# gillett-hernandez/rust-pathtracer

Measured on AMD Instinct MI355X. Metric: Msamples/s (paths×spp/s) Cornell box 1024², max_bounces=8; 1/2/4/8 GPU, higher is better.
Workload: dtype f32

## Files before the change

### include/pt_api.h

```cpp
#ifndef PT_API_H
#define PT_API_H

#include <stddef.h>
#include <stdint.h>

#ifdef __cplusplus
extern "C" {
#endif

typedef int32_t pt_status;
enum {
    PT_OK = 0,
    PT_ERR_INVALID_ARGUMENT = 1,
    PT_ERR_NO_DEVICE = 2,
    PT_ERR_OUT_OF_MEMORY = 3,
    PT_ERR_UNSUPPORTED = 4,
    PT_ERR_DEVICE = 5
};

enum { PT_TAG_MATERIAL = 0, PT_TAG_LIGHT = 1, PT_TAG_CAMERA = 2 };
#define PT_MATERIAL_ID(tag, index) ((((uint32_t)(tag)) << 16) | ((uint32_t)(index) & 0xffffu))
#define PT_MATERIAL_TAG(id) (((id) >> 16) & 0x3u)
#define PT_MATERIAL_INDEX(id) ((id) & 0xffffu)
#define PT_MATERIAL_NONE 0xffffffffu
// ... 152 lines not shown
    PT_TUNE_NO_CORE_LDS = 1u << 1,
    PT_TUNE_NO_PARK = 1u << 2,
    PT_TUNE_NO_LIVE_LIST = 1u << 3,
    PT_TUNE_EXACT_SLAB = 1u << 4,
    PT_TUNE_NO_CULL = 1u << 5,
    PT_TUNE_NO_SWEEP = 1u << 6,
    PT_TUNE_NO_MESH_SWEEP = 1u << 7,
    PT_TUNE_NO_KNOWN_LIGHT = 1u << 8,
    PT_TUNE_GENERAL_FORMS = 1u << 9,
    PT_TUNE_NO_FUSE = 1u << 10,
    PT_TUNE_NO_STAGE_TIMING = 1u << 11,
    PT_TUNE_MULTI_RCCL = 1u << 12,
    PT_TUNE_NO_ONE_LIGHT = 1u << 14,
    PT_TUNE_NO_CONVEX = 1u << 15,
    PT_TUNE_NO_MESH_SHORTCUTS = 1u << 16,
    PT_TUNE_NO_AXIS_SCAN = 1u << 13
};
typedef struct pt_tuning {
    uint32_t flags;
    uint32_t batch_slots;
    uint32_t blocks_per_cu;
    uint32_t park_blocks_per_cu;
    int32_t park_dynamic;
    uint32_t shade_form;
    uint32_t lds_all_limit;
    uint32_t multi_virtual;
    uint32_t walk_evict_below;
    uint32_t walk_search_below;
    uint32_t park_block;
    uint32_t light_prepass_max;
    uint32_t top_evict_below;
// ... 81 lines not shown
```

### rust-pathtracer_amd/api.py

```python
import ctypes as C
import numpy as np

PT_OK = 0
PT_ERR_UNSUPPORTED = 4
TAG_MATERIAL, TAG_LIGHT, TAG_CAMERA = 0, 1, 2
MATERIAL_NONE = 0xFFFFFFFF

CURVE_LINEAR, CURVE_TABULATED, CURVE_CAUCHY, CURVE_EXPONENTIAL, CURVE_INV_EXPONENTIAL, CURVE_BLACKBODY, CURVE_CONST = range(7)
INTERP_LINEAR, INTERP_NEAREST, INTERP_CUBIC = range(3)
TEXTURE1, TEXTURE4 = 1, 4
MATERIAL_LAMBERTIAN, MATERIAL_GGX, MATERIAL_DIFFUSE_LIGHT, MATERIAL_SHARP_LIGHT, MATERIAL_PASSTHROUGH = range(5)
MEDIUM_HG, MEDIUM_RAYLEIGH = range(2)
SIDED_FORWARD, SIDED_REVERSE, SIDED_DUAL = range(3)
SHAPE_RECT, SHAPE_SPHERE, SHAPE_DISK, SHAPE_MESH = range(4)
AXIS_X, AXIS_Y, AXIS_Z = range(3)
ENV_CONSTANT, ENV_SUN, ENV_HDR = range(3)


def material_id(tag, index):
    return ((tag & 3) << 16) | (index & 0xFFFF)


class Curve(C.Structure):
    _fields_ = [("kind", C.c_int32), ("mode", C.c_int32), ("p0", C.c_float), ("p1", C.c_float),
# ... 114 lines not shown
    _fields_ = [("max_chain", C.c_uint32), ("alpha_max", C.c_float), ("reserved", C.c_uint32 * 2)]


class Profile(C.Structure):
    _fields_ = [("bounce_rays", C.c_uint64), ("shadow_rays", C.c_uint64), ("light_rays", C.c_uint64),
                ("camera_rays", C.c_uint64), ("env_hits", C.c_uint64), ("seconds", C.c_double),
                ("kernel_seconds", C.c_double * 8), ("kernel_launches", C.c_uint64 * 8), ("stage_items", C.c_uint64 * 8)]

    def as_dict(self):
        return {"bounce_rays": self.bounce_rays, "shadow_rays": self.shadow_rays, "light_rays": self.light_rays,
                "camera_rays": self.camera_rays, "env_hits": self.env_hits, "seconds": self.seconds,
                "kernel_seconds": list(self.kernel_seconds), "kernel_launches": list(self.kernel_launches), "stage_items": list(self.stage_items)}


TUNE_NO_LDS, TUNE_NO_CORE_LDS, TUNE_NO_PARK, TUNE_NO_LIVE_LIST, TUNE_EXACT_SLAB, TUNE_NO_CULL, TUNE_NO_SWEEP, TUNE_NO_MESH_SWEEP, TUNE_NO_KNOWN_LIGHT, \
    TUNE_GENERAL_FORMS, TUNE_NO_FUSE, TUNE_NO_STAGE_TIMING, TUNE_MULTI_RCCL, TUNE_NO_AXIS_SCAN, TUNE_NO_ONE_LIGHT, TUNE_NO_CONVEX, TUNE_NO_MESH_SHORTCUTS = (1 << i for i in range(17))


class Tuning(C.Structure):
    _fields_ = [("flags", C.c_uint32), ("batch_slots", C.c_uint32), ("blocks_per_cu", C.c_uint32), ("park_blocks_per_cu", C.c_uint32),
                ("park_dynamic", C.c_int32), ("shade_form", C.c_uint32), ("lds_all_limit", C.c_uint32), ("multi_virtual", C.c_uint32),
                ("walk_evict_below", C.c_uint32), ("walk_search_below", C.c_uint32), ("park_block", C.c_uint32), ("light_prepass_max", C.c_uint32), ("top_evict_below", C.c_uint32), ("group_evict_below", C.c_uint32), ("reserved", C.c_uint32 * 2)]


class OutputDesc(C.Structure):
    _fields_ = [("width", C.c_uint32), ("height", C.c_uint32), ("tonemap", C.c_int32), ("luminance_only", C.c_int32),
                ("exposure", C.c_float), ("key_value", C.c_float), ("white_point", C.c_float), ("colorspace", C.c_int32),
                ("factor", C.c_float)]


TONEMAP_CLAMP, TONEMAP_REINHARD0, TONEMAP_REINHARD1 = range(3)
# ... 739 lines not shown
```

### rust-pathtracer_amd/csrc/pt_engine.hip

```cpp
#include <hip/hip_runtime.h>

#include <dlfcn.h>
#include <rccl/rccl.h>

#include <algorithm>
#include <chrono>
#include <condition_variable>
#include <functional>
#include <mutex>
#include <thread>
#include <cstdio>
#include <cstring>
#include <string>
#include <vector>

#include "pt_kernels.h"
#include "../../include/pt_adaptive.h"
#include "../../include/pt_spectral.h"
#include "../../include/pt_api.h"
#include "../../include/pt_debug.h"
#include "../../include/pt_denoise.h"
#include "pt_adaptive_select.h"
#include "pt_spectral_launch.h"
#include "pt_spectral_rules.h"
// ... 263 lines not shown
    }
    struct pt_resident_info info() const { struct pt_resident_info i; i.width = width; i.height = height; i.bins = bins; i.parts = parts; return i; }
};

struct pt_scene {
    pth::HostScene host;
    pt_tuning tuning;
    MultiSetup multi;
    uint32_t* d_blob = nullptr;
    float* d_tex = nullptr;
    uint32_t blob_words = 0;
    int lds_mode = 0;
    uint32_t lacks = 0;
    int device = 0, num_cus = 0;
    DeviceBuffers buf;
    AdaptiveBuffers adaptive;
    std::vector<hipEvent_t> events;
    GrowBuf film_cache;
    GrowBuf spectral_cache;
    bool spectral_valid = false;
    uint32_t spectral_width = 0, spectral_height = 0, spectral_bins = 0;
    std::vector<pt_scene*> spectral_shards;
    std::vector<uint32_t> shard_px;
    GrowBuf shard_packed;
    ResidentSet resident;
    GrowBuf assemble_staging, assemble_px;
    GrowBuf project_cache;
    std::vector<pt_scene*> replicas;
};

namespace {
bool scene_has_mesh(const std::vector<uint32_t>& blob) {
// ... 5 lines not shown
std::string g_device_info;

pt_status no_device() { return fail(PT_ERR_NO_DEVICE, "no HIP device available: the product path has no CPU fallback"); }
pt_status ensure_device() {
    int n = 0;
    hipError_t e = hipGetDeviceCount(&n);
    if (e != hipSuccess || n == 0) return no_device();
    return PT_OK;
}

uint32_t segment_capacity(uint32_t n, int grid) {
    uint32_t c = (n + (uint32_t)grid - 1) / (uint32_t)grid;
    return (c + 63u) & ~63u;
}

pt_status ensure_buffers(pt_scene* sc, uint32_t capacity, uint32_t light_samples, size_t n_pixels, int grid, uint32_t nl, uint32_t park_block) {
    DeviceBuffers& b = sc->buf;
    uint32_t total = segment_capacity(capacity, grid) * (uint32_t)grid;
    if (b.capacity < total || b.light_samples < light_samples || b.grid != grid || b.nl < nl || b.park_block < park_block) {
        hipFree(b.paths_a); hipFree(b.paths_b); hipFree(b.hits); hipFree(b.shadow); hipFree(b.energy); hipFree(b.counts); hipFree(b.block_stats); hipFree(b.park);
        b.paths_a = b.paths_b = b.hits = b.shadow = b.counts = b.park = nullptr; b.energy = nullptr; b.block_stats = nullptr; b.capacity = 0;
        uint32_t ls = light_samples > b.light_samples ? light_samples : b.light_samples;
        uint32_t nlmax = nl > b.nl ? nl : b.nl;
        size_t path_fields = nlmax == 4 ? Layout<4>::path_fields : Layout<1>::path_fields;
        size_t sh_fields = nlmax == 4 ? Layout<4>::shadow_queue_fields(ls ? ls : 1) : Layout<1>::shadow_queue_fields(ls ? ls : 1);
        HIP_TRY(hipMalloc(&b.paths_a, sizeof(uint32_t) * path_fields * total));
        HIP_TRY(hipMalloc(&b.paths_b, sizeof(uint32_t) * path_fields * total));
        HIP_TRY(hipMalloc(&b.hits, sizeof(uint32_t) * (size_t)HS_FIELDS * total));
        HIP_TRY(hipMalloc(&b.shadow, sizeof(uint32_t) * sh_fields * total));
        HIP_TRY(hipMalloc(&b.energy, sizeof(float) * (size_t)(nlmax + 1u) * total));
        b.nl = nlmax;
        HIP_TRY(hipMalloc(&b.counts, sizeof(uint32_t) * 4 * (size_t)grid));
        HIP_TRY(hipMalloc(&b.block_stats, sizeof(unsigned long long) * BS_FIELDS * (size_t)grid));
        const bool no_table = sc->host.blob[PT_HDR_SWEEP_OFF] == 0 || (sc->host.blob[PT_HDR_FLAGS] & PT_FLAG_NO_SWEEP);
        if ((sc->host.blob[PT_HDR_FLAGS] & PT_FLAG_SWEEP_WALKS) || no_table)
            HIP_TRY(hipMalloc(&b.park, sizeof(uint32_t) * kParkFields * (kParkCap / (kBlock / 64)) * (park_block / 64) * (size_t)grid));
        b.park_block = park_block;
        if (!b.unit_counters) HIP_TRY(hipMalloc(&b.unit_counters, sizeof(uint32_t) * kUnitCounters));
        b.capacity = total; b.light_samples = ls; b.grid = grid;
    }
    if (b.pixel_capacity < n_pixels) {
        hipFree(b.pixels); b.pixels = nullptr;
        HIP_TRY(hipMalloc(&b.pixels, sizeof(uint32_t) * n_pixels));
        b.pixel_capacity = n_pixels;
    }
    return PT_OK;
}

pt_status ensure_adaptive_buffers(pt_scene* sc, size_t n_pixels) {
    AdaptiveBuffers& a = sc->adaptive;
    if (a.pixels >= n_pixels) return PT_OK;
    a.release();
    const size_t blocks = (n_pixels + kBlock - 1) / kBlock;
    HIP_TRY(hipMalloc(&a.counts, sizeof(uint32_t) * n_pixels));
    HIP_TRY(hipMalloc(&a.lists[0], sizeof(uint32_t) * n_pixels));
// ... 194 lines not shown
                         : (env_prob != 0.0f || tn.shade_form == 2) ? PT_SHADE_FULL : (has_ggx || certs || tn.shade_form == 1) ? PT_SHADE_NO_ENV : PT_SHADE_LEAN;
    cfg.certs = certs;
    uint32_t live_list = ((trav_form == PT_FORM_SWEEP || trav_form == PT_FORM_WALK || trav_form == PT_FORM_ANY) && shade_form == PT_SHADE_LEAN && !(tn.flags & PT_TUNE_NO_LIVE_LIST)) ? 1u : 0u;
#ifdef PT_EXPERIMENTS
    if (cfg.live_lists || getenv("PT_AMD_EXP_SHADOW")) live_list = 0u;
#endif
    const uint32_t camera_record = (shade_form == PT_SHADE_LEAN || shade_form == PT_SHADE_FULL || shade_form == PT_SHADE_MEDIUM) ? 1u : 0u;
    cfg.fuse = !(tn.flags & PT_TUNE_NO_FUSE) && (!hero || PT_FUSE_HERO) && trav_form == PT_FORM_SWEEP && shade_form == PT_SHADE_LEAN && (cfg.lacks & PT_SCENE_NO_XF) != 0;
    const uint32_t path_fields = hero ? Layout<4>::path_fields : (rd.medium_aware ? (uint32_t)PS_FIELDS + 2u : Layout<1>::path_fields);
    const uint32_t item_fields = hero ? Layout<4>::shadow_queue_fields(rd.light_samples ? rd.light_samples : 1) : Layout<1>::shadow_queue_fields(rd.light_samples ? rd.light_samples : 1);
    *plan = RenderPlan{capacity, grid, hero, park_block, park_block_extend, trav_form, shade_form, park_dynamic, park_big, cfg, live_list, camera_record,
                       path_fields, item_fields};
    return PT_OK;
}

pt_status read_profile(pt_scene* sc, const RenderPlan& plan, uint64_t camera_rays, uint64_t accumulated_pixels, const double* stage_ms, const uint64_t* stage_launches,
                       uint32_t rounds, double seconds, pt_profile* profile) {
    memset(profile, 0, sizeof(*profile));
    std::vector<unsigned long long> bs((size_t)plan.grid * BS_FIELDS);
    HIP_TRY(hipMemcpy(bs.data(), sc->buf.block_stats, sizeof(unsigned long long) * bs.size(), hipMemcpyDeviceToHost));
    unsigned long long c[BS_FIELDS] = {0, 0, 0, 0, 0, 0};
    for (int g = 0; g < plan.grid; ++g) for (int k = 0; k < BS_FIELDS; ++k) c[k] += bs[(size_t)g * BS_FIELDS + k];
    profile->camera_rays = camera_rays;
    profile->bounce_rays = c[BS_VERTICES] + camera_rays;
    profile->shadow_rays = c[BS_SHADOW_RAYS];
    profile->env_hits = c[BS_ENV_HITS];
    profile->seconds = seconds;
    for (int i = 0; i < ST_COUNT; ++i) { profile->kernel_seconds[i] = stage_ms[i] * 1e-3; profile->kernel_launches[i] = stage_launches[i]; }
    profile->stage_items[ST_GENERATE] = camera_rays; profile->stage_items[ST_EXTEND] = c[BS_SEGMENTS]; profile->stage_items[ST_SHADE] = c[BS_SEGMENTS];
    profile->stage_items[ST_SHADOW] = c[BS_ITEMS]; profile->stage_items[ST_ACCUMULATE] = accumulated_pixels;
    profile->stage_items[6] = (uint64_t)plan.cfg.park_block;
    profile->stage_items[7] = plan.camera_record;
    profile->stage_items[5] = c[BS_MEDIUM_DROPS];
    profile->kernel_launches[5] = rounds;
    return PT_OK;
}

pt_status render_impl(pt_scene* sc, const pt_render_desc* rdp, float* d_film, hipStream_t stream, pt_profile* profile, const RenderJob& job) {
    if (!sc || !rdp || !d_film) return fail(PT_ERR_INVALID_ARGUMENT, "null argument");
    pt_render_desc rd;
    std::string err;
    if (!pth::normalize_render_desc(*rdp, (uint32_t)sc->host.cameras.size(), &rd, &err)) return fail(PT_ERR_INVALID_ARGUMENT, err);
    HIP_TRY(hipSetDevice(sc->device));

    const pt_adaptive_desc* adaptive = job.adaptive;
    std::vector<uint32_t> own_list;
    if (!job.shard_list) own_list = pth::shard_pixels(rd.width, rd.height, rd.tile_width, rd.tile_height, rd.shard_index, rd.shard_count);
    const std::vector<uint32_t>& pixels = job.shard_list ? *job.shard_list : own_list;
    RenderPlan plan;
    pt_status st = plan_render(sc, rd, job, pixels, stream, &plan);
    if (st != PT_OK) return st;
    const uint32_t capacity = plan.capacity;
    const int grid = plan.grid, trav_form = plan.trav_form, shade_form = plan.shade_form;
    const bool hero = plan.hero, park_dynamic = plan.park_dynamic;
    LaunchCfg cfg = plan.cfg;

    st = ensure_buffers(sc, capacity, rd.light_samples, pixels.size() ? pixels.size() : 1, grid, (hero || rd.medium_aware) ? 4u : 1u, plan.park_block);
    if (st != PT_OK) return st;
    DeviceBuffers& b = sc->buf;
    if ((trav_form == PT_FORM_PARKED || trav_form == PT_FORM_PARKED_WALK) && !b.park) return fail(PT_ERR_DEVICE, "internal: a parked traversal form without the parked kernels' scratch");
    if (adaptive) {
        const size_t film_pixels = (size_t)rd.width * rd.height;
        st = ensure_adaptive_buffers(sc, film_pixels);
        if (st != PT_OK) return st;
        if (!pixels.empty()) HIP_TRY(hipMemcpyAsync(sc->adaptive.lists[0], pixels.data(), sizeof(uint32_t) * pixels.size(), hipMemcpyHostToDevice, stream));
        if (job.shard_list && !pixels.empty()) HIP_TRY(hipMemcpyAsync(b.pixels, pixels.data(), sizeof(uint32_t) * pixels.size(), hipMemcpyHostToDevice, stream));
        HIP_TRY(hipMemsetAsync(sc->adaptive.stats, 0, sizeof(double) * 2 * film_pixels, stream));
        if (pixels.size() < film_pixels) HIP_TRY(hipMemsetAsync(sc->adaptive.counts, 0, sizeof(uint32_t) * film_pixels, stream));
    } else if (!pixels.empty()) HIP_TRY(hipMemcpyAsync(b.pixels, pixels.data(), sizeof(uint32_t) * pixels.size(), hipMemcpyHostToDevice, stream));
    HIP_TRY(hipMemsetAsync(d_film, 0, sizeof(float) * 4 * (size_t)rd.width * rd.height, stream));
    if (job.d_spectral) HIP_TRY(hipMemsetAsync(job.d_spectral, 0, sizeof(float) * (size_t)job.spectral_bins * rd.width * rd.height, stream));
    HIP_TRY(hipMemsetAsync(b.block_stats, 0, sizeof(unsigned long long) * BS_FIELDS * (size_t)grid, stream));

    RenderParams rp;
    memset(&rp, 0, sizeof(rp));
    rp.seed = rd.seed; rp.width = rd.width; rp.height = rd.height;
    rp.min_bounces = rd.min_bounces; rp.max_bounces = rd.max_bounces; rp.light_samples = rd.light_samples; rp.only_direct = rd.only_direct;
    rp.wavelength_lo = rd.wavelength_lo; rp.wavelength_span = rd.wavelength_hi - rd.wavelength_lo;
    rp.spp = adaptive ? adaptive->max_samples : rd.spp; rp.range_end = rd.first_sample + rd.sample_count;
    rp.normalize = (!adaptive && rd.first_sample == 0 && rd.sample_count == rd.spp) ? 1u : 0u;
    rp.phase = rd.phase_samples;
    rp.camera = pth::camera_params(sc->host.cameras[rd.camera_index], (float)rd.width / (float)rd.height);
    rp.energy_stride = b.capacity;
    rp.live_list = plan.live_list; rp.camera_record = plan.camera_record;

    const pt_tuning& tn = sc->tuning;
    const SceneArgs sargs{sc->d_blob, sc->blob_words, sc->d_tex, marginal_lds_bytes(sc->host.blob.data(), cfg.lds_bytes)};
    const uint32_t bounce_limit = rd.only_direct ? 1u : rd.max_bounces;
    const bool timing = !(tn.flags & PT_TUNE_NO_STAGE_TIMING);
    double stage_ms[ST_COUNT] = {0, 0, 0, 0, 0};
    uint64_t stage_launches[ST_COUNT] = {0, 0, 0, 0, 0};
    Queue qa{b.paths_a, b.capacity, plan.path_fields}, qb{b.paths_b, b.capacity, plan.path_fields}, qh{b.hits, b.capacity, HS_FIELDS}, qs{b.shadow, b.capacity, plan.item_fields};
    uint32_t* live[2] = {b.counts, b.counts + grid};
    uint32_t* nshadow = b.counts + 2 * grid;

    HIP_TRY(hipStreamSynchronize(stream));
    const auto t0 = std::chrono::steady_clock::now();
    std::vector<int> event_stage;
    auto event_at = [&](size_t k) -> bool {
        while (sc->events.size() <= k) { hipEvent_t e; if (hipEventCreate(&e) != hipSuccess) return false; sc->events.push_back(e); }
        return hipEventRecord(sc->events[k], stream) == hipSuccess;
    };
    bool events_ok = timing && event_at(0);
    auto timed = [&](int stage, auto&& fn) {
        fn();
        if (events_ok) { events_ok = event_at(event_stage.size() + 1); if (events_ok) event_stage.push_back(stage); }
        stage_launches[stage]++;
    };

    uint64_t camera_rays = 0, accumulated_pixels = 0;
    hipError_t spectral_error = hipSuccess;
    auto run_passes = [&](const uint32_t* d_list, uint32_t n_list, uint32_t first_sample, uint32_t sample_count, double* d_stats) -> pt_status {
        if (camera_rays != 0 && events_ok) { events_ok = event_at(event_stage.size() + 1); if (events_ok) event_stage.push_back(-1); }
        rp.range_end = first_sample + sample_count;
        std::vector<pth::Pass> passes = pth::plan_passes(n_list, first_sample, sample_count, capacity, rd.phase_samples);
        for (const pth::Pass& pass : passes) {
            accumulated_pixels += pass.pixel_count;
            rp.chunk_pixels = pass.pixel_count; rp.first_sample = pass.first_sample; rp.pass_samples = pass.sample_count;
            uint32_t n = pass.pixel_count * pass.sample_count;
            if (n > b.capacity) return fail(PT_ERR_DEVICE, "internal: a pass of " + std::to_string(n) + " slots exceeds the queue capacity " + std::to_string(b.capacity));
            uint32_t seg_cap = segment_capacity(n, grid);
            camera_rays += n;
            const uint32_t* d_px = d_list + pass.pixel_begin;
            if (park_dynamic) {
                HIP_TRY(hipMemsetAsync(b.unit_counters, 0, sizeof(uint32_t) * kUnitCounters, stream));
                if (events_ok) { events_ok = event_at(event_stage.size() + 1); if (events_ok) event_stage.push_back(-1); }
            }
            timed(ST_GENERATE, [&] {
                if (hero) hipLaunchKernelGGL(k_generate<4>, dim3(grid), dim3(kBlock), 0, stream, rp, d_px, qa, b.energy, n, seg_cap, live[0]);
                else hipLaunchKernelGGL(k_generate<1>, dim3(grid), dim3(kBlock), 0, stream, rp, d_px, qa, b.energy, n, seg_cap, live[0]);
            });
            for (uint32_t bounce = 0; bounce < bounce_limit; ++bounce) {
                Queue qin = (bounce & 1) ? qb : qa, qout = (bounce & 1) ? qa : qb;
                uint32_t *cin = live[bounce & 1], *cout = live[(bounce + 1) & 1];
                if (park_dynamic) cfg.unit_counter = b.unit_counters + 2 * bounce;
                cfg.path_marks = (bounce > 0 && !rd.medium_aware && (sc->host.blob[PT_HDR_FLAGS] & PT_FLAG_CONVEX)) ? sc->host.blob[PT_HDR_CONVEX_INST] : 0u;
                if (!cfg.fuse) timed(ST_EXTEND, [&] { launch_extend(cfg, trav_form, sargs, qin, qh, seg_cap, cin, b.park); });
                if (park_dynamic) cfg.unit_counter = b.unit_counters + 2 * bounce + 1;
                timed(ST_SHADE, [&] { launch_shade(cfg, hero ? 4 : 1, shade_form, sargs, rp, bounce, d_px, qin, qh, qout, qs, b.energy, seg_cap, cin, cout, nshadow, b.block_stats); });
                if (rd.light_samples > 0)
                    timed(ST_SHADOW, [&] { launch_shadow(cfg, trav_form, hero ? 4 : 1, shade_form == PT_SHADE_FULL || shade_form == PT_SHADE_MEDIUM, sargs, rd.light_samples, qs, b.energy, b.capacity, rp.live_list ? (seg_cap | kShadowListed) : seg_cap, nshadow, b.park, qh); });
            }
            timed(ST_ACCUMULATE, [&] {
                if (d_stats && hero) hipLaunchKernelGGL(k_accumulate_stats<4>, dim3(grid), dim3(kBlock), 0, stream, rp, d_px, b.energy, d_film, d_stats);
                else if (d_stats) hipLaunchKernelGGL(k_accumulate_stats<1>, dim3(grid), dim3(kBlock), 0, stream, rp, d_px, b.energy, d_film, d_stats);
                else if (hero) hipLaunchKernelGGL(k_accumulate<4>, dim3(grid), dim3(kBlock), 0, stream, rp, d_px, b.energy, d_film);
                else hipLaunchKernelGGL(k_accumulate<1>, dim3(grid), dim3(kBlock), 0, stream, rp, d_px, b.energy, d_film);
                if (job.d_spectral && spectral_error == hipSuccess)
                    spectral_error = ptk::launch_accumulate_spectral(hero ? 4 : 1, grid, stream, rp, d_px, b.energy, job.d_spectral, job.spectral_bins, rd.width * rd.height);
            });
            if (spectral_error != hipSuccess) return fail(PT_ERR_DEVICE, std::string("k_accumulate_spectral: ") + hipGetErrorString(spectral_error));
        }
        return PT_OK;
    };
    uint32_t rounds = 0;
    st = adaptive ? adaptive_rounds(sc, rd, *adaptive, stream, d_film, (uint32_t)pixels.size(), run_passes, &rounds, job.node, job.node_index)
                  : run_passes(b.pixels, (uint32_t)pixels.size(), rd.first_sample, rd.sample_count, nullptr);
    if (st != PT_OK) return st;
    if (adaptive && job.d_spectral)
        hipLaunchKernelGGL(k_adaptive_finish_spectral, dim3(sc->num_cus * 4), dim3(kBlock), 0, stream, rd.width * rd.height, job.spectral_bins, sc->adaptive.counts, job.d_spectral);
    HIP_TRY(hipGetLastError());
    HIP_TRY(hipStreamSynchronize(stream));
    auto t1 = std::chrono::steady_clock::now();
    for (size_t k = 0; k < event_stage.size(); ++k) {
        float ms = 0.0f;
        if (event_stage[k] >= 0 && hipEventElapsedTime(&ms, sc->events[k], sc->events[k + 1]) == hipSuccess) stage_ms[event_stage[k]] += ms;
    }
    if (profile) return read_profile(sc, plan, camera_rays, accumulated_pixels, stage_ms, stage_launches, rounds, std::chrono::duration<double>(t1 - t0).count(), profile);
    return PT_OK;
}

pt_status probe_material(pt_scene* sc, int mode, uint32_t record, size_t n, const float* lambda, const float* a, size_t a_w, const float* b, size_t b_w,
                         float* f, float* wo, float* pdf) {
    HIP_TRY(hipSetDevice(sc->device));
    DevBuf dl, da, db, df, dwo, dp;
    size_t m = n ? n : 1;
    HIP_TRY(dl.alloc(4 * m)); HIP_TRY(da.alloc(4 * m * 3)); HIP_TRY(db.alloc(4 * m * 3));
    HIP_TRY(df.alloc(4 * m)); HIP_TRY(dwo.alloc(4 * m * 3)); HIP_TRY(dp.alloc(4 * m));
    HIP_TRY(hipMemcpy(dl.p, lambda, 4 * n, hipMemcpyHostToDevice));
    if (a) HIP_TRY(hipMemcpy(da.p, a, 4 * n * a_w, hipMemcpyHostToDevice));
    if (b) HIP_TRY(hipMemcpy(db.p, b, 4 * n * b_w, hipMemcpyHostToDevice));
    hipLaunchKernelGGL(k_probe_material, dim3(256), dim3(kBlock), 0, 0, sc->d_blob, sc->d_tex, mode, record, (uint32_t)n, dl.as<float>(), da.as<float>(), db.as<float>(),
                       df.as<float>(), dwo.as<float>(), dp.as<float>());
// ... 71 lines not shown
    }
    return PT_OK;
}

void pt_tuning_default(pt_tuning* t) {
    if (!t) return;
    memset(t, 0, sizeof(*t));
    const struct { const char* name; uint32_t bit; } flags[] = {
        {"PT_AMD_NO_LDS", PT_TUNE_NO_LDS}, {"PT_AMD_NO_CORE_LDS", PT_TUNE_NO_CORE_LDS}, {"PT_AMD_NO_PARK", PT_TUNE_NO_PARK},
#ifdef PT_EXPERIMENTS
        {"PT_AMD_POOL", PT_TUNE_EXPERIMENT_POOL},
#endif

        {"PT_AMD_EXACT_SLAB", PT_TUNE_EXACT_SLAB}, {"PT_AMD_NO_CULL", PT_TUNE_NO_CULL}, {"PT_AMD_NO_SWEEP", PT_TUNE_NO_SWEEP}, {"PT_AMD_NO_MESH_SWEEP", PT_TUNE_NO_MESH_SWEEP},
        {"PT_AMD_NO_KNOWN_LIGHT", PT_TUNE_NO_KNOWN_LIGHT}, {"PT_AMD_GENERAL_FORMS", PT_TUNE_GENERAL_FORMS}, {"PT_AMD_NO_FUSE", PT_TUNE_NO_FUSE}, {"PT_AMD_MULTI_RCCL", PT_TUNE_MULTI_RCCL}, {"PT_AMD_NO_AXIS_SCAN", PT_TUNE_NO_AXIS_SCAN}, {"PT_AMD_NO_ONE_LIGHT", PT_TUNE_NO_ONE_LIGHT}, {"PT_AMD_NO_CONVEX", PT_TUNE_NO_CONVEX}, {"PT_AMD_NO_MESH_SHORTCUTS", PT_TUNE_NO_MESH_SHORTCUTS},
        {"PT_AMD_NO_LIVE_LIST", PT_TUNE_NO_LIVE_LIST},
    };
    for (const auto& f : flags) if (env_u32(f.name, 0)) t->flags |= f.bit;
    if (env_u32("PT_AMD_STAGE_TIMING", 1) == 0) t->flags |= PT_TUNE_NO_STAGE_TIMING;
    t->batch_slots = env_u32("PT_AMD_BATCH", 0);
    t->blocks_per_cu = env_u32("PT_AMD_BLOCKS_PER_CU", 0);
    t->park_blocks_per_cu = env_u32("PT_AMD_PARK_BLOCKS_PER_CU", 0);
    t->park_dynamic = getenv("PT_AMD_PARK_DYNAMIC") && *getenv("PT_AMD_PARK_DYNAMIC") ? (env_u32("PT_AMD_PARK_DYNAMIC", 0) != 0 ? 1 : 0) : -1;
    t->shade_form = env_u32("PT_AMD_SHADE_FORM", 0);
    t->lds_all_limit = env_u32("PT_AMD_LDS_ALL_LIMIT", 0);
    t->multi_virtual = env_u32("PT_AMD_MULTI_VIRTUAL", 0);
    t->walk_evict_below = env_u32("PT_AMD_WALK_EVICT_BELOW", 0);
    t->walk_search_below = env_u32("PT_AMD_WALK_SEARCH_BELOW", 0);
    t->park_block = env_u32("PT_AMD_PARK_BLOCK", 0);
    t->light_prepass_max = env_u32("PT_AMD_LIGHT_PREPASS_MAX", 0);
    t->top_evict_below = env_u32("PT_AMD_TOP_EVICT_BELOW", 0);
    t->group_evict_below = env_u32("PT_AMD_GROUP_EVICT_BELOW", 0);
}

pt_status pt_scene_create(const pt_scene_desc* desc, pt_scene** out) {
    pt_tuning t;
    pt_tuning_default(&t);
    return pt_scene_create_tuned(desc, &t, out);
}

pt_status pt_scene_create_tuned(const pt_scene_desc* desc, const pt_tuning* tuning, pt_scene** out) {
    if (!desc || !out || !tuning) return fail(PT_ERR_INVALID_ARGUMENT, "null argument");
    for (uint32_t r : tuning->reserved) if (r != 0) return fail(PT_ERR_INVALID_ARGUMENT, "pt_tuning::reserved must be 0");
    if (tuning->park_block != 0 && tuning->park_block != 256 && tuning->park_block != 512 && tuning->park_block != 1024)
        return fail(PT_ERR_INVALID_ARGUMENT, "pt_tuning::park_block (PT_AMD_PARK_BLOCK) must be 0, 256, 512 or 1024");
    if (tuning->shade_form > 2 || tuning->park_dynamic < -1 || tuning->park_dynamic > 1 || tuning->multi_virtual > 64 || tuning->walk_evict_below > 64 || tuning->walk_search_below > 64 || tuning->top_evict_below > 64 || tuning->group_evict_below > 64)
        return fail(PT_ERR_INVALID_ARGUMENT, "pt_tuning: shade_form in 0..2, park_dynamic in -1..1, multi_virtual, walk_evict_below, walk_search_below, top_evict_below, group_evict_below <= 64");
// ... 8 lines not shown
    st = scene_to_device(sc);
    if (st != PT_OK) { const std::string msg = g_error; pt_scene_destroy(sc); g_error = msg; return st; }
    *out = sc;
    return PT_OK;
}

static void multi_release(MultiSetup& m);
static void forget_node_render(pt_scene* sc) { if (sc) sc->multi.node_render = NodeRemembered(); }
void pt_scene_destroy(pt_scene* sc) {
    if (!sc) return;
    for (pt_scene* r : sc->replicas) if (r) pt_scene_destroy(r);
    sc->replicas.clear();
    if (sc->multi.valid) multi_release(sc->multi);
    hipSetDevice(sc->device);
    sc->buf.release();
    sc->adaptive.release();
    hipFree(sc->d_blob); hipFree(sc->d_tex);
    for (auto& e : sc->events) hipEventDestroy(e);
    delete sc;
}

pt_status pt_render_device(pt_scene* sc, const pt_render_desc* rd, void* film_device, void* hip_stream, pt_profile* profile) {
    return render_impl(sc, rd, static_cast<float*>(film_device), static_cast<hipStream_t>(hip_stream), profile, RenderJob());
}

struct RenderCall {
    const pt_render_desc* rd = nullptr;
    const pt_adaptive_desc* ad = nullptr;
    const pt_spectral_desc* sd = nullptr;
    float* film = nullptr;
    uint32_t* sample_counts = nullptr;
    double* stats = nullptr;
    float* spectral = nullptr;
// ... 1007 lines not shown
```

### rust-pathtracer_amd/csrc/pt_plan.cpp

```cpp
#include "pt_plan.h"
#include "pt_denoise_rules.h"
#include "pt_guides_chain_rules.h"

#include <cmath>
#include <cstring>

namespace pth {

std::vector<uint32_t> shard_pixels(uint32_t width, uint32_t height, uint32_t tw, uint32_t th, uint32_t shard_index, uint32_t shard_count) {
    struct T { uint32_t x0, x1, y0, y1; };
    std::vector<T> tiles;
    uint32_t fx = width / tw, fy = height / th, rx = width % tw, ry = height % th;
    for (uint32_t y = 0; y < fy; ++y) for (uint32_t x = 0; x < fx; ++x) tiles.push_back(T{x * tw, x * tw + tw, y * th, y * th + th});
    if (rx) for (uint32_t y = 0; y < fy; ++y) tiles.push_back(T{fx * tw, fx * tw + rx, y * th, y * th + th});
    if (ry) {
        for (uint32_t x = 0; x < fx; ++x) tiles.push_back(T{x * tw, x * tw + tw, fy * th, fy * th + ry});
        if (rx) tiles.push_back(T{fx * tw, fx * tw + rx, fy * th, fy * th + ry});
    }
    std::vector<uint32_t> mine;
    for (size_t t = 0; t < tiles.size(); ++t)
        if (!shard_count || PT_TILE_SHARD((uint32_t)t, fx, shard_count) == shard_index) mine.push_back((uint32_t)t);
    const size_t n = mine.size();
    size_t stride = (size_t)((double)n * 0.3819660112501051);
    auto gcd = [](size_t a, size_t b) { while (b) { size_t t = a % b; a = b; b = t; } return a; };
    if (stride < 1) stride = 1;
    while (gcd(stride, n ? n : 1) != 1) ++stride;
    std::vector<uint32_t> px;
    for (size_t i = 0; i < n; ++i) {
        const T& tile = tiles[mine[(i * stride) % n]];
        for (uint32_t y = tile.y0; y < tile.y1; ++y)
            for (uint32_t x = tile.x0; x < tile.x1; ++x) px.push_back(y * width + x);
    }
    return px;
}

std::vector<Pass> plan_passes(uint32_t n_pixels, uint32_t first_sample, uint32_t sample_count, uint32_t capacity, uint32_t phase_samples) {
    std::vector<Pass> passes;
    if (n_pixels == 0 || sample_count == 0) return passes;
    const uint32_t period = phase_samples ? phase_samples : 10;
    uint32_t phase = sample_count < period ? sample_count : period;
    uint32_t max_chunk = capacity / phase;
    if (max_chunk == 0) max_chunk = 1;
    uint32_t n_chunks = (n_pixels + max_chunk - 1) / max_chunk;
    uint32_t chunk = (n_pixels + n_chunks - 1) / n_chunks;
    for (uint32_t p0 = 0; p0 < n_pixels; p0 += chunk) {
        uint32_t pc = (n_pixels - p0 < chunk) ? n_pixels - p0 : chunk;
        uint32_t max_s = capacity / pc;
        if (max_s < phase) max_s = phase;
// ... 386 lines not shown
```

### rust-pathtracer_amd/csrc/pt_plan.h

```cpp
#ifndef PT_PLAN_H
#define PT_PLAN_H
#include <stdint.h>

#include <string>
#include <vector>

#include "../../include/pt_adaptive.h"
#include "../../include/pt_api.h"
#include "../../include/pt_denoise.h"
#include "../../include/pt_resident.h"
#include "../../include/pt_spectral.h"
#include "pt_stages.h"

namespace pth {

std::vector<uint32_t> shard_pixels(uint32_t width, uint32_t height, uint32_t tile_w, uint32_t tile_h,
                                   uint32_t shard_index, uint32_t shard_count);

struct Pass { uint32_t pixel_begin, pixel_count, first_sample, sample_count; };
std::vector<Pass> plan_passes(uint32_t n_pixels, uint32_t first_sample, uint32_t sample_count, uint32_t capacity, uint32_t phase_samples = 10);

ptd::CameraParams camera_params(const pt_camera& c, float aspect_ratio);

bool normalize_render_desc(const pt_render_desc& in, uint32_t camera_count, pt_render_desc* out, std::string* error);
pt_status normalize_adaptive_desc(const pt_render_desc& in, const pt_adaptive_desc& adaptive, bool has_sample_counts, uint32_t camera_count,
                                  pt_render_desc* out, pt_adaptive_desc* adaptive_out, std::string* error);

pt_status normalize_denoise_desc(const pt_denoise_desc* in, const void* film, const void* sample_counts, const void* stats, const void* guides, const void* out_film,
                                 pt_denoise_desc* out, std::string* error);
pt_status check_denoise_inputs(const pt_denoise_desc& d, const uint32_t* sample_counts, const float* guides, std::string* error);
pt_status check_guides_args(const void* scene, const pt_render_desc* rd, uint32_t camera_count, uint32_t guide_samples, const void* guides, std::string* error);
pt_status check_denoise_albedo(const pt_denoise_desc& d, const float* albedo, std::string* error);
pt_status check_albedo_basis_args(const pt_render_desc* rd, const void* lambda, const void* xyz, std::string* error);
pt_status check_guides_chain_args(const void* scene, const pt_render_desc* rd, uint32_t camera_count, uint32_t guide_samples, const pt_guide_chain_desc* chain,
                                  const void* guides, pt_guide_chain_desc* out, std::string* error);
// ... 46 lines not shown
```

Before: 2390.

## Overlap consecutive render passes on a second stream with double-buffered queues

Adds a second set of device buffers and a non-blocking stream so consecutive wavefront passes alternate between two lanes. A pass may start once the previous pass reaches a configurable skew bounce, and accumulation is serialized with events, so the tail of one pass (few live paths, low occupancy) overlaps the head of the next. It also skips allocating the hit queue when extend and shade are fused. The cost is double scratch memory, extra event synchronization, and two passes contending for the GPU at once.

```diff
diff --git a/include/pt_api.h b/include/pt_api.h
--- a/include/pt_api.h
+++ b/include/pt_api.h
@@ -190,7 +190,10 @@
     PT_TUNE_NO_ONE_LIGHT = 1u << 14,
     PT_TUNE_NO_CONVEX = 1u << 15,
     PT_TUNE_NO_MESH_SHORTCUTS = 1u << 16,
-    PT_TUNE_NO_AXIS_SCAN = 1u << 13
+    PT_TUNE_NO_AXIS_SCAN = 1u << 13,
+    PT_TUNE_NO_PASS_OVERLAP = 1u << 17,
+    PT_TUNE_PASS_SKEW_SHIFT = 18,
+    PT_TUNE_PASS_SKEW_MASK = 7
 };
 typedef struct pt_tuning {
     uint32_t flags;
diff --git a/rust-pathtracer_amd/api.py b/rust-pathtracer_amd/api.py
--- a/rust-pathtracer_amd/api.py
+++ b/rust-pathtracer_amd/api.py
@@ -152,7 +152,9 @@
 
 
 TUNE_NO_LDS, TUNE_NO_CORE_LDS, TUNE_NO_PARK, TUNE_NO_LIVE_LIST, TUNE_EXACT_SLAB, TUNE_NO_CULL, TUNE_NO_SWEEP, TUNE_NO_MESH_SWEEP, TUNE_NO_KNOWN_LIGHT, \
-    TUNE_GENERAL_FORMS, TUNE_NO_FUSE, TUNE_NO_STAGE_TIMING, TUNE_MULTI_RCCL, TUNE_NO_AXIS_SCAN, TUNE_NO_ONE_LIGHT, TUNE_NO_CONVEX, TUNE_NO_MESH_SHORTCUTS = (1 << i for i in range(17))
+    TUNE_GENERAL_FORMS, TUNE_NO_FUSE, TUNE_NO_STAGE_TIMING, TUNE_MULTI_RCCL, TUNE_NO_AXIS_SCAN, TUNE_NO_ONE_LIGHT, TUNE_NO_CONVEX, TUNE_NO_MESH_SHORTCUTS, \
+    TUNE_NO_PASS_OVERLAP = (1 << i for i in range(18))
+TUNE_PASS_SKEW_SHIFT, TUNE_PASS_SKEW_MASK = 18, 7
 
 
 class Tuning(C.Structure):
diff --git a/rust-pathtracer_amd/csrc/pt_engine.hip b/rust-pathtracer_amd/csrc/pt_engine.hip
--- a/rust-pathtracer_amd/csrc/pt_engine.hip
+++ b/rust-pathtracer_amd/csrc/pt_engine.hip
@@ -301,8 +301,11 @@
     uint32_t lacks = 0;
     int device = 0, num_cus = 0;
     DeviceBuffers buf;
+    DeviceBuffers buf2;
+    hipStream_t pass_stream = nullptr;
+    std::vector<hipEvent_t> pass_deps;
     AdaptiveBuffers adaptive;
-    std::vector<hipEvent_t> events;
+    std::vector<hipEvent_t> events, events2;
     GrowBuf film_cache;
     GrowBuf spectral_cache;
     bool spectral_valid = false;
@@ -338,8 +341,7 @@
     return (c + 63u) & ~63u;
 }
 
-pt_status ensure_buffers(pt_scene* sc, uint32_t capacity, uint32_t light_samples, size_t n_pixels, int grid, uint32_t nl, uint32_t park_block) {
-    DeviceBuffers& b = sc->buf;
+pt_status ensure_buffers(pt_scene* sc, DeviceBuffers& b, uint32_t capacity, uint32_t light_samples, size_t n_pixels, int grid, uint32_t nl, uint32_t park_block, bool need_hits) {
     uint32_t total = segment_capacity(capacity, grid) * (uint32_t)grid;
     if (b.capacity < total || b.light_samples < light_samples || b.grid != grid || b.nl < nl || b.park_block < park_block) {
         hipFree(b.paths_a); hipFree(b.paths_b); hipFree(b.hits); hipFree(b.shadow); hipFree(b.energy); hipFree(b.counts); hipFree(b.block_stats); hipFree(b.park);
@@ -350,7 +352,6 @@
         size_t sh_fields = nlmax == 4 ? Layout<4>::shadow_queue_fields(ls ? ls : 1) : Layout<1>::shadow_queue_fields(ls ? ls : 1);
         HIP_TRY(hipMalloc(&b.paths_a, sizeof(uint32_t) * path_fields * total));
         HIP_TRY(hipMalloc(&b.paths_b, sizeof(uint32_t) * path_fields * total));
-        HIP_TRY(hipMalloc(&b.hits, sizeof(uint32_t) * (size_t)HS_FIELDS * total));
         HIP_TRY(hipMalloc(&b.shadow, sizeof(uint32_t) * sh_fields * total));
         HIP_TRY(hipMalloc(&b.energy, sizeof(float) * (size_t)(nlmax + 1u) * total));
         b.nl = nlmax;
@@ -363,6 +364,7 @@
         if (!b.unit_counters) HIP_TRY(hipMalloc(&b.unit_counters, sizeof(uint32_t) * kUnitCounters));
         b.capacity = total; b.light_samples = ls; b.grid = grid;
     }
+    if (need_hits && !b.hits) HIP_TRY(hipMalloc(&b.hits, sizeof(uint32_t) * (size_t)HS_FIELDS * b.capacity));
     if (b.pixel_capacity < n_pixels) {
         hipFree(b.pixels); b.pixels = nullptr;
         HIP_TRY(hipMalloc(&b.pixels, sizeof(uint32_t) * n_pixels));
@@ -587,13 +589,16 @@
     return PT_OK;
 }
 
-pt_status read_profile(pt_scene* sc, const RenderPlan& plan, uint64_t camera_rays, uint64_t accumulated_pixels, const double* stage_ms, const uint64_t* stage_launches,
+pt_status read_profile(pt_scene* sc, const RenderPlan& plan, bool second_set, uint64_t camera_rays, uint64_t accumulated_pixels, const double* stage_ms, const uint64_t* stage_launches,
                        uint32_t rounds, double seconds, pt_profile* profile) {
     memset(profile, 0, sizeof(*profile));
     std::vector<unsigned long long> bs((size_t)plan.grid * BS_FIELDS);
-    HIP_TRY(hipMemcpy(bs.data(), sc->buf.block_stats, sizeof(unsigned long long) * bs.size(), hipMemcpyDeviceToHost));
     unsigned long long c[BS_FIELDS] = {0, 0, 0, 0, 0, 0};
-    for (int g = 0; g < plan.grid; ++g) for (int k = 0; k < BS_FIELDS; ++k) c[k] += bs[(size_t)g * BS_FIELDS + k];
+    for (const unsigned long long* d_bs : {(const unsigned long long*)sc->buf.block_stats, (const unsigned long long*)(second_set ? sc->buf2.block_stats : nullptr)}) {
+        if (!d_bs) continue;
+        HIP_TRY(hipMemcpy(bs.data(), d_bs, sizeof(unsigned long long) * bs.size(), hipMemcpyDeviceToHost));
+        for (int g = 0; g < plan.grid; ++g) for (int k = 0; k < BS_FIELDS; ++k) c[k] += bs[(size_t)g * BS_FIELDS + k];
+    }
     profile->camera_rays = camera_rays;
     profile->bounce_rays = c[BS_VERTICES] + camera_rays;
     profile->shadow_rays = c[BS_SHADOW_RAYS];
@@ -609,6 +614,8 @@
     return PT_OK;
 }
 
+enum { DEP_FORK = 0, DEP_ACCUMULATED = 1, DEP_SKEW = 3, DEP_COUNT = 5 };
+
 pt_status render_impl(pt_scene* sc, const pt_render_desc* rdp, float* d_film, hipStream_t stream, pt_profile* profile, const RenderJob& job) {
     if (!sc || !rdp || !d_film) return fail(PT_ERR_INVALID_ARGUMENT, "null argument");
     pt_render_desc rd;
@@ -628,9 +635,31 @@
     const bool hero = plan.hero, park_dynamic = plan.park_dynamic;
     LaunchCfg cfg = plan.cfg;
 
-    st = ensure_buffers(sc, capacity, rd.light_samples, pixels.size() ? pixels.size() : 1, grid, (hero || rd.medium_aware) ? 4u : 1u, plan.park_block);
+#ifdef PT_EXPERIMENTS
+    const bool need_hits = true;
+#else
+    const bool need_hits = !cfg.fuse;
+#endif
+    st = ensure_buffers(sc, sc->buf, capacity, rd.light_samples, pixels.size() ? pixels.size() : 1, grid, (hero || rd.medium_aware) ? 4u : 1u, plan.park_block, need_hits);
     if (st != PT_OK) return st;
     DeviceBuffers& b = sc->buf;
+    bool overlap = !(sc->tuning.flags & PT_TUNE_NO_PASS_OVERLAP);
+    if (overlap) {
+        const uint32_t n_px = (uint32_t)pixels.size();
+        overlap = pth::plan_passes(n_px, rd.first_sample, adaptive ? rd.spp : rd.sample_count, capacity, rd.phase_samples).size() >= 2
+               || (adaptive && adaptive->max_samples > rd.spp && pth::plan_passes(n_px, rd.spp, adaptive->step < adaptive->max_samples - rd.spp ? adaptive->step : adaptive->max_samples - rd.spp, capacity, rd.phase_samples).size() >= 2);
+    }
+    if (overlap) {
+        bool ok = ensure_buffers(sc, sc->buf2, capacity, rd.light_samples, 0, grid, (hero || rd.medium_aware) ? 4u : 1u, plan.park_block, need_hits) == PT_OK;
+        if (ok && !sc->pass_stream) ok = hipStreamCreateWithFlags(&sc->pass_stream, hipStreamNonBlocking) == hipSuccess;
+        while (ok && sc->pass_deps.size() < DEP_COUNT) {
+            hipEvent_t e;
+            ok = hipEventCreateWithFlags(&e, hipEventDisableTiming) == hipSuccess;
+            if (ok) sc->pass_deps.push_back(e);
+        }
+        if (!ok) { sc->buf2.release(); (void)hipGetLastError(); overlap = false; }
+    }
+    if (overlap && (trav_form == PT_FORM_PARKED || trav_form == PT_FORM_PARKED_WALK) && !sc->buf2.park) return fail(PT_ERR_DEVICE, "internal: a parked traversal form without the second set's scratch");
     if ((trav_form == PT_FORM_PARKED || trav_form == PT_FORM_PARKED_WALK) && !b.park) return fail(PT_ERR_DEVICE, "internal: a parked traversal form without the parked kernels' scratch");
     if (adaptive) {
         const size_t film_pixels = (size_t)rd.width * rd.height;
@@ -644,6 +673,7 @@
     HIP_TRY(hipMemsetAsync(d_film, 0, sizeof(float) * 4 * (size_t)rd.width * rd.height, stream));
     if (job.d_spectral) HIP_TRY(hipMemsetAsync(job.d_spectral, 0, sizeof(float) * (size_t)job.spectral_bins * rd.width * rd.height, stream));
     HIP_TRY(hipMemsetAsync(b.block_stats, 0, sizeof(unsigned long long) * BS_FIELDS * (size_t)grid, stream));
+    if (overlap) HIP_TRY(hipMemsetAsync(sc->buf2.block_stats, 0, sizeof(unsigned long long) * BS_FIELDS * (size_t)grid, stream));
 
     RenderParams rp;
     memset(&rp, 0, sizeof(rp));
@@ -654,7 +684,6 @@
     rp.normalize = (!adaptive && rd.first_sample == 0 && rd.sample_count == rd.spp) ? 1u : 0u;
     rp.phase = rd.phase_samples;
     rp.camera = pth::camera_params(sc->host.cameras[rd.camera_index], (float)rd.width / (float)rd.height);
-    rp.energy_stride = b.capacity;
     rp.live_list = plan.live_list; rp.camera_record = plan.camera_record;
 
     const pt_tuning& tn = sc->tuning;
@@ -663,31 +692,61 @@
     const bool timing = !(tn.flags & PT_TUNE_NO_STAGE_TIMING);
     double stage_ms[ST_COUNT] = {0, 0, 0, 0, 0};
     uint64_t stage_launches[ST_COUNT] = {0, 0, 0, 0, 0};
-    Queue qa{b.paths_a, b.capacity, plan.path_fields}, qb{b.paths_b, b.capacity, plan.path_fields}, qh{b.hits, b.capacity, HS_FIELDS}, qs{b.shadow, b.capacity, plan.item_fields};
-    uint32_t* live[2] = {b.counts, b.counts + grid};
-    uint32_t* nshadow = b.counts + 2 * grid;
+    struct Lane {
+        DeviceBuffers* set; hipStream_t stream; std::vector<hipEvent_t>* events;
+        Queue qa, qb, qh, qs;
+        uint32_t* live[2];
+        uint32_t* nshadow;
+        size_t marks;
+        std::vector<int> stage;
+    };
+    auto make_lane = [&](DeviceBuffers& s, hipStream_t on, std::vector<hipEvent_t>* ev) {
+        return Lane{&s, on, ev, Queue{s.paths_a, s.capacity, plan.path_fields}, Queue{s.paths_b, s.capacity, plan.path_fields}, Queue{s.hits, s.capacity, HS_FIELDS},
+                    Queue{s.shadow, s.capacity, plan.item_fields}, {s.counts, s.counts + grid}, s.counts + 2 * grid, 0, {}};
+    };
+    Lane lanes[2] = {make_lane(b, stream, &sc->events), make_lane(overlap ? sc->buf2 : b, overlap ? sc->pass_stream : stream, &sc->events2)};
 
     HIP_TRY(hipStreamSynchronize(stream));
     const auto t0 = std::chrono::steady_clock::now();
-    std::vector<int> event_stage;
-    auto event_at = [&](size_t k) -> bool {
-        while (sc->events.size() <= k) { hipEvent_t e; if (hipEventCreate(&e) != hipSuccess) return false; sc->events.push_back(e); }
-        return hipEventRecord(sc->events[k], stream) == hipSuccess;
+    bool events_ok = timing;
+    auto mark = [&](Lane& l, int stage) {
+        if (!events_ok) return;
+        while (l.events->size() <= l.marks) { hipEvent_t e; if (hipEventCreate(&e) != hipSuccess) { events_ok = false; return; } l.events->push_back(e); }
+        if (hipEventRecord((*l.events)[l.marks], l.stream) != hipSuccess) { events_ok = false; return; }
+        if (l.marks > 0) l.stage.push_back(stage);
+        ++l.marks;
     };
-    bool events_ok = timing && event_at(0);
-    auto timed = [&](int stage, auto&& fn) {
+    mark(lanes[0], -1);
+    auto timed = [&](Lane& l, int stage, auto&& fn) {
         fn();
-        if (events_ok) { events_ok = event_at(event_stage.size() + 1); if (events_ok) event_stage.push_back(stage); }
+        mark(l, stage);
         stage_launches[stage]++;
     };
 
     uint64_t camera_rays = 0, accumulated_pixels = 0;
     hipError_t spectral_error = hipSuccess;
+    bool overlapped = false;
+    const std::vector<hipEvent_t>& dep = sc->pass_deps;
+    const uint32_t skew_code = (tn.flags >> PT_TUNE_PASS_SKEW_SHIFT) & PT_TUNE_PASS_SKEW_MASK;
+    const int32_t skew_bounce = skew_code == 0u ? pth::kPassSkewBounce : (int32_t)skew_code - 2;
     auto run_passes = [&](const uint32_t* d_list, uint32_t n_list, uint32_t first_sample, uint32_t sample_count, double* d_stats) -> pt_status {
-        if (camera_rays != 0 && events_ok) { events_ok = event_at(event_stage.size() + 1); if (events_ok) event_stage.push_back(-1); }
+        if (camera_rays != 0) mark(lanes[0], -1);
         rp.range_end = first_sample + sample_count;
         std::vector<pth::Pass> passes = pth::plan_passes(n_list, first_sample, sample_count, capacity, rd.phase_samples);
-        for (const pth::Pass& pass : passes) {
+        const pth::PassSchedule sch = pth::schedule_passes((uint32_t)passes.size(), bounce_limit, skew_bounce, overlap);
+        const bool two_lanes = sch.steps.size() >= 2 && sch.steps[1].lane == 1u;
+        if (two_lanes) { HIP_TRY(hipEventRecord(dep[DEP_FORK], stream)); overlapped = true; }
+        for (size_t p = 0; p < passes.size(); ++p) {
+            const pth::Pass& pass = passes[p];
+            const pth::PassStep& step = sch.steps[p];
+            Lane& l = lanes[step.lane];
+            DeviceBuffers& b = *l.set;
+            const hipStream_t stream = l.stream;
+            const Queue &qa = l.qa, &qb = l.qb, &qh = l.qh, &qs = l.qs;
+            uint32_t* const* live = l.live;
+            uint32_t* const nshadow = l.nshadow;
+            cfg.stream = stream;
+            rp.energy_stride = b.capacity;
             accumulated_pixels += pass.pixel_count;
             rp.chunk_pixels = pass.pixel_count; rp.first_sample = pass.first_sample; rp.pass_samples = pass.sample_count;
             uint32_t n = pass.pixel_count * pass.sample_count;
@@ -695,11 +754,14 @@
             uint32_t seg_cap = segment_capacity(n, grid);
             camera_rays += n;
             const uint32_t* d_px = d_list + pass.pixel_begin;
+            if (step.wait_fork) HIP_TRY(hipStreamWaitEvent(stream, dep[DEP_FORK], 0));
+            if (step.start_after >= 0) HIP_TRY(hipStreamWaitEvent(stream, dep[DEP_SKEW + (step.start_after & 1)], 0));
+            if (step.wait_fork || step.start_after >= 0) mark(l, -1);
             if (park_dynamic) {
                 HIP_TRY(hipMemsetAsync(b.unit_counters, 0, sizeof(uint32_t) * kUnitCounters, stream));
-                if (events_ok) { events_ok = event_at(event_stage.size() + 1); if (events_ok) event_stage.push_back(-1); }
+                mark(l, -1);
             }
-            timed(ST_GENERATE, [&] {
+            timed(l, ST_GENERATE, [&] {
                 if (hero) hipLaunchKernelGGL(k_generate<4>, dim3(grid), dim3(kBlock), 0, stream, rp, d_px, qa, b.energy, n, seg_cap, live[0]);
                 else hipLaunchKernelGGL(k_generate<1>, dim3(grid), dim3(kBlock), 0, stream, rp, d_px, qa, b.energy, n, seg_cap, live[0]);
             });
@@ -708,13 +770,15 @@
                 uint32_t *cin = live[bounce & 1], *cout = live[(bounce + 1) & 1];
                 if (park_dynamic) cfg.unit_counter = b.unit_counters + 2 * bounce;
                 cfg.path_marks = (bounce > 0 && !rd.medium_aware && (sc->host.blob[PT_HDR_FLAGS] & PT_FLAG_CONVEX)) ? sc->host.blob[PT_HDR_CONVEX_INST] : 0u;
-                if (!cfg.fuse) timed(ST_EXTEND, [&] { launch_extend(cfg, trav_form, sargs, qin, qh, seg_cap, cin, b.park); });
+                if (!cfg.fuse) timed(l, ST_EXTEND, [&] { launch_extend(cfg, trav_form, sargs, qin, qh, seg_cap, cin, b.park); });
                 if (park_dynamic) cfg.unit_counter = b.unit_counters + 2 * bounce + 1;
-                timed(ST_SHADE, [&] { launch_shade(cfg, hero ? 4 : 1, shade_form, sargs, rp, bounce, d_px, qin, qh, qout, qs, b.energy, seg_cap, cin, cout, nshadow, b.block_stats); });
+                timed(l, ST_SHADE, [&] { launch_shade(cfg, hero ? 4 : 1, shade_form, sargs, rp, bounce, d_px, qin, qh, qout, qs, b.energy, seg_cap, cin, cout, nshadow, b.block_stats); });
                 if (rd.light_samples > 0)
-                    timed(ST_SHADOW, [&] { launch_shadow(cfg, trav_form, hero ? 4 : 1, shade_form == PT_SHADE_FULL || shade_form == PT_SHADE_MEDIUM, sargs, rd.light_samples, qs, b.energy, b.capacity, rp.live_list ? (seg_cap | kShadowListed) : seg_cap, nshadow, b.park, qh); });
+                    timed(l, ST_SHADOW, [&] { launch_shadow(cfg, trav_form, hero ? 4 : 1, shade_form == PT_SHADE_FULL || shade_form == PT_SHADE_MEDIUM, sargs, rd.light_samples, qs, b.energy, b.capacity, rp.live_list ? (seg_cap | kShadowListed) : seg_cap, nshadow, b.park, qh); });
+                if ((int32_t)bounce == step.signal_bounce) HIP_TRY(hipEventRecord(dep[DEP_SKEW + (p & 1)], stream));
             }
-            timed(ST_ACCUMULATE, [&] {
+            if (step.accumulate_after >= 0) { HIP_TRY(hipStreamWaitEvent(stream, dep[DEP_ACCUMULATED + (step.accumulate_after & 1)], 0)); mark(l, -1); }
+            timed(l, ST_ACCUMULATE, [&] {
                 if (d_stats && hero) hipLaunchKernelGGL(k_accumulate_stats<4>, dim3(grid), dim3(kBlock), 0, stream, rp, d_px, b.energy, d_film, d_stats);
                 else if (d_stats) hipLaunchKernelGGL(k_accumulate_stats<1>, dim3(grid), dim3(kBlock), 0, stream, rp, d_px, b.energy, d_film, d_stats);
                 else if (hero) hipLaunchKernelGGL(k_accumulate<4>, dim3(grid), dim3(kBlock), 0, stream, rp, d_px, b.energy, d_film);
@@ -723,7 +787,9 @@
                     spectral_error = ptk::launch_accumulate_spectral(hero ? 4 : 1, grid, stream, rp, d_px, b.energy, job.d_spectral, job.spectral_bins, rd.width * rd.height);
             });
             if (spectral_error != hipSuccess) return fail(PT_ERR_DEVICE, std::string("k_accumulate_spectral: ") + hipGetErrorString(spectral_error));
+            if (two_lanes) HIP_TRY(hipEventRecord(dep[DEP_ACCUMULATED + (p & 1)], stream));
         }
+        if (sch.join_pass >= 0) HIP_TRY(hipStreamWaitEvent(stream, dep[DEP_ACCUMULATED + (sch.join_pass & 1)], 0));
         return PT_OK;
     };
     uint32_t rounds = 0;
@@ -735,11 +801,20 @@
     HIP_TRY(hipGetLastError());
     HIP_TRY(hipStreamSynchronize(stream));
     auto t1 = std::chrono::steady_clock::now();
-    for (size_t k = 0; k < event_stage.size(); ++k) {
+    for (const Lane& l : lanes) for (size_t k = 0; k < l.stage.size(); ++k) {
         float ms = 0.0f;
-        if (event_stage[k] >= 0 && hipEventElapsedTime(&ms, sc->events[k], sc->events[k + 1]) == hipSuccess) stage_ms[event_stage[k]] += ms;
-    }
-    if (profile) return read_profile(sc, plan, camera_rays, accumulated_pixels, stage_ms, stage_launches, rounds, std::chrono::duration<double>(t1 - t0).count(), profile);
+        if (l.stage[k] >= 0 && hipEventElapsedTime(&ms, (*l.events)[k], (*l.events)[k + 1]) == hipSuccess) stage_ms[l.stage[k]] += ms;
+    }
+    if (overlapped && lanes[0].marks > 0) {
+        double window = 0.0, total = 0.0;
+        for (const Lane& l : lanes) {
+            float ms = 0.0f;
+            if (l.marks > 0 && hipEventElapsedTime(&ms, (*lanes[0].events)[0], (*l.events)[l.marks - 1]) == hipSuccess && ms > window) window = ms;
+        }
+        for (double ms : stage_ms) total += ms;
+        if (window > 0.0 && total > window) for (double& ms : stage_ms) ms *= window / total;
+    }
+    if (profile) return read_profile(sc, plan, overlap, camera_rays, accumulated_pixels, stage_ms, stage_launches, rounds, std::chrono::duration<double>(t1 - t0).count(), profile);
     return PT_OK;
 }
 
@@ -841,7 +916,7 @@
 
         {"PT_AMD_EXACT_SLAB", PT_TUNE_EXACT_SLAB}, {"PT_AMD_NO_CULL", PT_TUNE_NO_CULL}, {"PT_AMD_NO_SWEEP", PT_TUNE_NO_SWEEP}, {"PT_AMD_NO_MESH_SWEEP", PT_TUNE_NO_MESH_SWEEP},
         {"PT_AMD_NO_KNOWN_LIGHT", PT_TUNE_NO_KNOWN_LIGHT}, {"PT_AMD_GENERAL_FORMS", PT_TUNE_GENERAL_FORMS}, {"PT_AMD_NO_FUSE", PT_TUNE_NO_FUSE}, {"PT_AMD_MULTI_RCCL", PT_TUNE_MULTI_RCCL}, {"PT_AMD_NO_AXIS_SCAN", PT_TUNE_NO_AXIS_SCAN}, {"PT_AMD_NO_ONE_LIGHT", PT_TUNE_NO_ONE_LIGHT}, {"PT_AMD_NO_CONVEX", PT_TUNE_NO_CONVEX}, {"PT_AMD_NO_MESH_SHORTCUTS", PT_TUNE_NO_MESH_SHORTCUTS},
-        {"PT_AMD_NO_LIVE_LIST", PT_TUNE_NO_LIVE_LIST},
+        {"PT_AMD_NO_LIVE_LIST", PT_TUNE_NO_LIVE_LIST}, {"PT_AMD_NO_PASS_OVERLAP", PT_TUNE_NO_PASS_OVERLAP},
     };
     for (const auto& f : flags) if (env_u32(f.name, 0)) t->flags |= f.bit;
     if (env_u32("PT_AMD_STAGE_TIMING", 1) == 0) t->flags |= PT_TUNE_NO_STAGE_TIMING;
@@ -858,6 +933,7 @@
     t->light_prepass_max = env_u32("PT_AMD_LIGHT_PREPASS_MAX", 0);
     t->top_evict_below = env_u32("PT_AMD_TOP_EVICT_BELOW", 0);
     t->group_evict_below = env_u32("PT_AMD_GROUP_EVICT_BELOW", 0);
+    t->flags |= (env_u32("PT_AMD_PASS_SKEW", 0) & PT_TUNE_PASS_SKEW_MASK) << PT_TUNE_PASS_SKEW_SHIFT;
 }
 
 pt_status pt_scene_create(const pt_scene_desc* desc, pt_scene** out) {
@@ -896,9 +972,11 @@
     if (sc->multi.valid) multi_release(sc->multi);
     hipSetDevice(sc->device);
     sc->buf.release();
+    sc->buf2.release();
     sc->adaptive.release();
     hipFree(sc->d_blob); hipFree(sc->d_tex);
-    for (auto& e : sc->events) hipEventDestroy(e);
+    for (auto* list : {&sc->events, &sc->events2, &sc->pass_deps}) for (auto& e : *list) hipEventDestroy(e);
+    if (sc->pass_stream) hipStreamDestroy(sc->pass_stream);
     delete sc;
 }
 
diff --git a/rust-pathtracer_amd/csrc/pt_plan.cpp b/rust-pathtracer_amd/csrc/pt_plan.cpp
--- a/rust-pathtracer_amd/csrc/pt_plan.cpp
+++ b/rust-pathtracer_amd/csrc/pt_plan.cpp
@@ -32,6 +32,23 @@
             for (uint32_t x = tile.x0; x < tile.x1; ++x) px.push_back(y * width + x);
     }
     return px;
+}
+
+PassSchedule schedule_passes(uint32_t n_passes, uint32_t bounces, int32_t skew_bounce, bool overlap) {
+    PassSchedule sch;
+    sch.steps.assign(n_passes, PassStep{0u, false, -1, -1, -1});
+    if (!overlap || n_passes < 2) return sch;
+    const int32_t g = (skew_bounce < 0 || bounces == 0) ? -1 : (skew_bounce < (int32_t)bounces ? skew_bounce : (int32_t)bounces - 1);
+    for (uint32_t p = 0; p < n_passes; ++p) {
+        PassStep& s = sch.steps[p];
+        s.lane = p & 1u;
+        s.wait_fork = p == 1;
+        s.start_after = (p > 0 && g >= 0) ? (int32_t)p - 1 : -1;
+        s.accumulate_after = p > 0 ? (int32_t)p - 1 : -1;
+        s.signal_bounce = p + 1 < n_passes ? g : -1;
+    }
+    sch.join_pass = ((n_passes - 1) & 1u) ? (int32_t)n_passes - 1 : -1;
+    return sch;
 }
 
 std::vector<Pass> plan_passes(uint32_t n_pixels, uint32_t first_sample, uint32_t sample_count, uint32_t capacity, uint32_t phase_samples) {
diff --git a/rust-pathtracer_amd/csrc/pt_plan.h b/rust-pathtracer_amd/csrc/pt_plan.h
--- a/rust-pathtracer_amd/csrc/pt_plan.h
+++ b/rust-pathtracer_amd/csrc/pt_plan.h
@@ -19,6 +19,11 @@
 
 struct Pass { uint32_t pixel_begin, pixel_count, first_sample, sample_count; };
 std::vector<Pass> plan_passes(uint32_t n_pixels, uint32_t first_sample, uint32_t sample_count, uint32_t capacity, uint32_t phase_samples = 10);
+
+struct PassStep { uint32_t lane; bool wait_fork; int32_t start_after, accumulate_after, signal_bounce; };
+struct PassSchedule { std::vector<PassStep> steps; int32_t join_pass = -1; };
+PassSchedule schedule_passes(uint32_t n_passes, uint32_t bounces, int32_t skew_bounce, bool overlap);
+constexpr int32_t kPassSkewBounce = 0;
 
 ptd::CameraParams camera_params(const pt_camera& c, float aspect_ratio);
 
```

Result: faster. 2471 (median of 6 runs) (+3.4%).
